# jedison-github/gentun

Measured on AMD Instinct MI355X. Metric: candidates/hour + best val-acc@genN, Genetic-CNN CIFAR-10 1/2/4/8 GPU, higher is better.
Workload: dtype fp32

## Files before the change

### csrc/hip/cnn_args.h

```cpp
#pragma once
#include "common.h"

template <typename F>
static void lds_limit(F* fn, size_t bytes) {
  if (bytes > 65536) (void)hipFuncSetAttribute(reinterpret_cast<const void*>(fn), hipFuncAttributeMaxDynamicSharedMemorySize,
                                         (int)bytes);
}

struct GroupRec {
  int g;
  int in_mask;
  int out_mask;
  int pad;
};

#define GT_MAXSLOT 8

struct ConvArgs {
  const void* in[GT_MAXSLOT];
  const void* mask;
  const int64_t* gather;
  const StepState* st;
  void* out[GT_MAXSLOT];
  const void* out_mask[GT_MAXSLOT];
// ... 17 lines not shown
  int Hr, Wr;
  int wino;
  int wfrag;
  int twopass;
};

__device__ __forceinline__ GroupRec group_rec(const GroupRec* gtab, int y, int n_in, int n_out, int acc,
                                              const void* const* out_mask) {
  if (gtab) return gtab[y];
  GroupRec r;
  r.g = y;
  r.in_mask = (1 << n_in) - 1;
  int rm = 0;
  for (int k = 0; k < n_out; ++k)
    if (out_mask && out_mask[k]) rm |= 1 << k;
  r.out_mask = ((1 << n_out) - 1) | ((acc & 0xff) << 8) | (rm << 16);
  r.pad = 0;
  return r;
}

struct WgradArgs {
  const void* in[GT_MAXSLOT];
  const int64_t* gather;
  const StepState* st;
  const void* dz;
  float* part_w;
  float* part_b;
  const GroupRec* gtab;
  int n_in;
  int G, B, H, W, Cinp, Coutp, KH, KW, S, pps;
  int ngroups;
  int prec;
  int cout_real;
};

__device__ __forceinline__ bool pos_bits(uint32_t h) { return h != 0u && h < 0x8000u; }
```

### csrc/hip/cnn_conv_fast.hip

```cpp
#include "conv_fast_host.h"

FastSwitches g_fast;

static int swap_switch(int& sw, int v) {
  const int old = sw;
  sw = v;
  return old;
}

extern "C" int gt_conv_set_s2in_ct1(int on) { return swap_switch(g_fast.s2in_ct1, on); }

extern "C" int gt_conv_set_regepi(int on) { return swap_switch(g_fast.regepi, on); }

extern "C" int gt_conv_set_smallq(int on) { return swap_switch(g_fast.smallq, on); }

static int smallq_th(const ConvArgs* a, int TH, int THMIN) {
  if (!g_fast.smallq) return TH;
  int th = TH;
  while (th > THMIN && (long)a->ngroups * a->B * (a->H / th) < g_fast.smallq_wg) th >>= 1;
  return th;
}

static bool pk_ok(const ConvArgs* a, int nt) {
  const int last = a->cout_real - 16 * (nt - 1);
// ... 158 lines not shown
      float acc = 0.f;
      for (int sp = 0; sp < a.S; ++sp) acc += pb[(long)sp * a.G * a.Coutp + i];
      pb[i] = acc;
    }
  }
}

extern "C" int gt_wgrad_reduce(const WgradArgs* a, hipStream_t stream) {
  const long n = (long)a->Coutp * a->KH * a->KW * a->Cinp;
  if (n % 4 || a->S < 2) return -1;
  dim3 grid((unsigned)((n / 4 + 255) / 256), a->ngroups);
  hipLaunchKernelGGL(wgrad_reduce_kernel, grid, dim3(256), 0, stream, *a);
  return (int)hipGetLastError();
}

extern "C" int gt_wgrad_set_nb(int nb) { return swap_switch(g_fast.wgrad_nb, nb); }

extern "C" int gt_wgrad_set_nz(int nz) { return swap_switch(g_fast.wgrad_nz, nz); }

static int wgrad_nz(const WgradArgs* a) {
  const int force = g_fast.wgrad_nz;
  if (force == 1 || force == 2 || force == 4 || force == 8) return force;
  const int blocks = a->S * a->ngroups;
  return blocks < 64 ? 4 : blocks < 160 ? 2 : 1;
}

static bool wgrad_pk_ok(const WgradArgs* a, int mt) {
  const int last = a->cout_real - 16 * (mt - 1);
  return a->cout_real > 0 && last >= 1 && last <= 4;
}

static const std::vector<WgradRow>& wgrad_rows() {
  static const std::vector<WgradRow> rows = {
    wgrad_f32<5, 5, 1, 3, 32, 8, 4, 1>(),
    wgrad_f32<3, 3, 3, 3, 32, 4, 4, 1>(),
    wgrad_f32<5, 5, 3, 7, 16, 4, 8, 1>(),
    wgrad_f32<3, 3, 7, 7, 16, 4, 8, 1>(),
    wgrad_f32z<5, 5, 7, 13, 8, 4, 8, 4>(),
    wgrad_f32z<3, 3, 13, 13, 8, 4, 8, 4>(),
    wgrad_f32<5, 5, 1, 8, 32, 4, 4, 1>(),
    wgrad_f32<3, 3, 8, 8, 32, 2, 8, 1>(),
    wgrad_f32z<5, 5, 8, 16, 16, 2, 8, 7>(),
    wgrad_f32z<3, 3, 16, 16, 16, 2, 8, 4>(),
    wgrad_f32z<5, 5, 16, 32, 8, 4, 8, 13>(),
    wgrad_f32z<3, 3, 32, 32, 8, 4, 8, 10>(),
    wgrad_bf16<5, 5, 1, 3, 32, 8, 4, 1>(),
    wgrad_bf16<3, 3, 3, 3, 32, 8, 4, 1>(),
    wgrad_bf16<5, 5, 3, 7, 16, 16, 8, 2>(),
    wgrad_bf16<3, 3, 7, 7, 16, 16, 8, 2>(),
  };
  return rows;
}

static const WgradRow* wgrad_row(int KH, int KW, int Cinp, int Coutp, int H, int W, int prec) {
  for (const std::vector<WgradRow>* rows : {&wgrad_rows(), &wgrad_rows_ext()})
    for (const WgradRow& r : *rows)
      if (KH == r.KH && KW == r.KW && Cinp == r.NCBI * 8 && Coutp == r.NCBO * 8 && W == r.W && prec == r.PREC &&
          H % r.R == 0)
        return &r;
  return nullptr;
}

struct WgradChoice {
  const WgradKernel* k;
  dim3 grid;
  unsigned block;
};

static bool select_wgrad(const WgradArgs* a, WgradChoice* c) {
  const WgradRow* r = wgrad_row(a->KH, a->KW, a->Cinp, a->Coutp, a->H, a->W, a->prec);
  if (!r || a->pps % (r->R * r->W) != 0) return false;
  const int nz = r->NZ ? r->NZ : wgrad_nz(a);
  const int pk = r->PREC == 1 && wgrad_pk_ok(a, (r->NCBO * 8 + 15) / 16) ? 1 : 0;
  int nw = r->NW, nb = 1;
  if (r->NZ == 0 && nz == 2) nb = r->NB;
  else if (r->NZ == 0 && nz == 8) nw = 4;
  else if (nz == 1) nb = (g_fast.wgrad_nb ? g_fast.wgrad_nb : r->NB) == 1 ? 1 : 2;
  for (const WgradKernel& k : r->k)
    if (k.NW == nw && k.NB == nb && k.PK == pk && k.NZ == nz) {
      *c = {&k, dim3(a->S, a->ngroups, nz), (unsigned)nw * 64};
      return true;
    }
  return false;
}

extern "C" int gt_wgrad_fast_band(int KH, int KW, int Cinp, int Coutp, int H, int W, int prec) {
  const WgradRow* r = wgrad_row(KH, KW, Cinp, Coutp, H, W, prec);
  return r ? r->R * r->W : 0;
}

extern "C" int gt_wgrad_fast_splits(int KH, int KW, int Cinp, int Coutp, int H, int W, int prec) {
  (void)KH; (void)KW; (void)Cinp; (void)Coutp; (void)H;
  if (prec == 1) {
    return W >= 32 ? 32 : W <= 8 ? 4 : 8;
  }
  return W >= 32 ? 16 : 3;
}

extern "C" int gt_wgrad_fast(const WgradArgs* a, hipStream_t stream) {
  if (a->prec != 0 && a->prec != 1) return -1;
  WgradChoice c;
  if (!select_wgrad(a, &c)) return -100;
  return launch_fast(c.k->fn, c.grid, c.block, 0, a, stream);
}

struct WgradSel {
  int KH, KW, NCBI, NCBO, W, R, NW, NB, PK, NZ, PREC;
  int gx, gy, gz, block, lds;
};
extern "C" int gt_wgrad_fast_select(const WgradArgs* a, WgradSel* s) {
  WgradChoice c;
  if (!select_wgrad(a, &c)) return 0;
  const WgradKernel& k = *c.k;
  *s = {k.KH, k.KW, k.NCBI, k.NCBO, k.W, k.R, k.NW, k.NB, k.PK, k.NZ, k.PREC,
        (int)c.grid.x, (int)c.grid.y, (int)c.grid.z, (int)c.block, 0};
  return 1;
}
extern "C" size_t gt_sizeof_wgrad_sel() { return sizeof(WgradSel); }

extern "C" int gt_conv_frag_order(int KH, int KW, int NCBI, int W, int prec, int* out, int n) {
  const int NCH = KH * KW * NCBI;
  const bool parts = prec == 1 && NCBI == 7 && W == 16 && KH == 3 && KW == 3;
  for (int e = 0; e < n; ++e) {
    int kk, cb;
    if (e >= NCH) { out[e] = -1; continue; }
    if (parts) {
      const int E0 = KH * KW * 4;
      if (e < E0) { kk = e >> 2; cb = e & 3; }
      else { const int e1 = e - E0; kk = e1 / 3; cb = 4 + e1 - kk * 3; }
    } else {
      kk = e / NCBI; cb = e - kk * NCBI;
    }
    out[e] = kk * NCBI + cb;
  }
  return (NCH + 3) / 4;
}

struct FragSeg {
  const float* w;
  uint16_t* dst;
  const int* order;
  long ps;
  int Q, Cop, Cip, KH, KW;
  int NT, NKS, NCBIc;
  int dgrad;
  int npl;
};

struct FragArgs {
  const FragSeg* segs;
  const int2* blocks;
// ... 51 lines not shown
```

### csrc/hip/conv_fast_host.h

```cpp
#pragma once
#include <initializer_list>
#include <vector>

#include "conv_fast_impl.h"

struct FastSwitches {
  int s2in_ct1 = 1;
  int regepi = 1;
  int smallq = 1;
  long smallq_wg = 300;
  int wgrad_nb = 0;
  int wgrad_nz = 0;
};
extern FastSwitches g_fast;

struct ConvKernel {
  int KH, KW, NCBI, W, TH, NT, NCO, NWV, PREC, PK, RE, CTX, SCH;
  int lds_fwd, lds_bwd;
  int TWO;
  const void* fn;
};

template <int KH, int KW, int NCBI, int W, int TH, int NT, int NCO, int NWV, int PREC, int PK = 0, int RE = 0,
          int CTX = 0, int SCH = 0, int TWO = 0>
// ... 12 lines not shown
  IF_TWO = 16,
};

struct ConvVariant {
  int cond;
  ConvKernel k;
};
typedef std::vector<ConvVariant> ConvVariants;

template <int KH, int KW, int NCBI, int W, int TH, int NT, int NCO, int NWV, int PREC, int PK = 0>
static ConvVariants tile(int cond = 0) {
  ConvVariants v;
  if (PREC == 1 && W % 16 == 0) v.push_back({cond | IF_RE, conv_kernel<KH, KW, NCBI, W, TH, NT, NCO, NWV, PREC, PK, 1>()});
  v.push_back({cond, conv_kernel<KH, KW, NCBI, W, TH, NT, NCO, NWV, PREC, PK, 0>()});
  return v;
}

template <int KH, int KW, int NCBI, int W, int TH, int NT, int NCO, int NWV, int SCH = 1, int TWO = 0>
static ConvVariants ct1(int cond = 0) {
  return {{cond, conv_kernel<KH, KW, NCBI, W, TH, NT, NCO, NWV, 1, 0, 1, 1, SCH, TWO>()}};
}

struct ConvRow {
  int hmod, thmin;
  ConvVariants v;
  ConvRow(int hmod_, int thmin_, std::initializer_list<ConvVariants> parts) : hmod(hmod_), thmin(thmin_) {
    for (const ConvVariants& p : parts) v.insert(v.end(), p.begin(), p.end());
  }
};

struct WgradKernel {
  int KH, KW, NCBI, NCBO, W, R, NW, NB, PK, NZ, PREC;
  const void* fn;
};

template <int KH, int KW, int NCBI, int NCBO, int W, int R, int NW, int NB, int PK = 0, int NZ = 1>
static WgradKernel wgrad_kernel_f32() {
  return {KH, KW, NCBI, NCBO, W, R, NW, NB, PK, NZ, 1,
          reinterpret_cast<const void*>(&wgrad_fast_f32_kernel<KH, KW, NCBI, NCBO, W, R, NW, NB, PK, NZ>)};
}
template <int KH, int KW, int NCBI, int NCBO, int W, int R, int NW, int NB>
static WgradKernel wgrad_kernel_bf16() {
  return {KH, KW, NCBI, NCBO, W, R, NW, NB, 0, 1, 0,
          reinterpret_cast<const void*>(&wgrad_fast_kernel<KH, KW, NCBI, NCBO, W, R, NW, NB>)};
}

struct WgradRow {
  int KH, KW, NCBI, NCBO, W, R, NW, PREC;
  int NB;
  int NZ;
  std::vector<WgradKernel> k;
};

template <int KH, int KW, int NCBI, int NCBO, int W, int R, int NW, int NB>
static WgradRow wgrad_f32() {
  return {KH, KW, NCBI, NCBO, W, R, NW, 1, NB, 0,
          {wgrad_kernel_f32<KH, KW, NCBI, NCBO, W, R, NW, 1, 0>(), wgrad_kernel_f32<KH, KW, NCBI, NCBO, W, R, NW, 1, 1>(),
           wgrad_kernel_f32<KH, KW, NCBI, NCBO, W, R, NW, 2, 0>(), wgrad_kernel_f32<KH, KW, NCBI, NCBO, W, R, NW, 2, 1>(),
           wgrad_kernel_f32<KH, KW, NCBI, NCBO, W, R, NW, NB, 0, 2>(), wgrad_kernel_f32<KH, KW, NCBI, NCBO, W, R, NW, NB, 1, 2>(),
           wgrad_kernel_f32<KH, KW, NCBI, NCBO, W, R, NW, 1, 0, 4>(), wgrad_kernel_f32<KH, KW, NCBI, NCBO, W, R, NW, 1, 1, 4>(),
           wgrad_kernel_f32<KH, KW, NCBI, NCBO, W, R, 4, 1, 0, 8>(), wgrad_kernel_f32<KH, KW, NCBI, NCBO, W, R, 4, 1, 1, 8>()}};
}
template <int KH, int KW, int NCBI, int NCBO, int W, int R, int NW, int NZ>
static WgradRow wgrad_f32z() {
  return {KH, KW, NCBI, NCBO, W, R, NW, 1, 1, NZ,
          {wgrad_kernel_f32<KH, KW, NCBI, NCBO, W, R, NW, 1, 0, NZ>(), wgrad_kernel_f32<KH, KW, NCBI, NCBO, W, R, NW, 1, 1, NZ>()}};
}
template <int KH, int KW, int NCBI, int NCBO, int W, int R, int NW, int NB>
static WgradRow wgrad_bf16() {
  return {KH, KW, NCBI, NCBO, W, R, NW, 0, NB, 1,
          {wgrad_kernel_bf16<KH, KW, NCBI, NCBO, W, R, NW, 1>(), wgrad_kernel_bf16<KH, KW, NCBI, NCBO, W, R, NW, 2>()}};
}

const std::vector<ConvRow>& conv_rows_ext();
const std::vector<WgradRow>& wgrad_rows_ext();
```

### csrc/hip/conv_fast_impl.h

```cpp
#pragma once

#include <algorithm>
#include <cstdio>
#include <cstdlib>
#include <type_traits>

#include "cnn_args.h"


__device__ __forceinline__ int opaque_i(int x) {
  asm volatile("" : "+v"(x));
  return x;
}

template <int KH, int KW, int NCBI, int W, int PREC>
struct S2Parts {
  static constexpr bool on = PREC == 1 && NCBI == 7 && W == 16 && KH == 3 && KW == 3;
  static constexpr int e0 = KH * KW * 4;
};

template <int KH, int KW, int NCBI, int W, int TH, int NT, int NCO, int PREC, int TWO = 0>
struct FastCfg {
  static_assert(!TWO || S2Parts<KH, KW, NCBI, W, PREC>::on, "two-pass staging follows the part-major order");
  static constexpr int NPL = PREC ? GT_NPL_F32 : 1;
// ... 864 lines not shown
        uint4 bfr = tr_pair(x0, x0 + 4 * XROW);
        if (n == NCH / 2 && ones_lane) bfr = make_uint4(0x3f803f80u, 0x3f803f80u, 0x3f803f80u, 0x3f803f80u);
#pragma unroll
        for (int m = 0; m < MT; ++m) acc[m][t] = mfma16(afr[m], bfr, acc[m][t]);
      }
    }
    if (NB == 1 && band + 1 < band1) {
      __syncthreads();
      issue(band + 1, 0);
    }
  }

  const int kq = lane >> 4;
  constexpr int Kdim = NCH * 8;
#pragma unroll
  for (int t = 0; t < TPW; ++t) {
    const int n = wave + NW * t;
    if (n >= NKT) continue;
    const int col = n * 16 + l16;
#pragma unroll
    for (int m = 0; m < MT; ++m)
#pragma unroll
      for (int i = 0; i < 4; ++i) {
        const int co = m * 16 + kq * 4 + i;
        if (co >= a.Coutp) continue;
        if (col < Kdim)
          a.part_w[(((long)s * a.G + g) * a.Coutp + co) * Kdim + col] = acc[m][t][i];
        else if (col == Kdim && a.part_b)
          a.part_b[((long)s * a.G + g) * a.Coutp + co] = acc[m][t][i];
      }
  }
}

template <int KH, int KW, int NCBI, int NCBO, int W, int R, int NW, int NB, int PK = 0, int NZ = 1>
__global__ void __launch_bounds__(NW * 64) wgrad_fast_f32_kernel(WgradArgs a) {
  constexpr int NPL = GT_NPL_F32;
  constexpr int NT_ = NW * 64;
  constexpr int PW = W + KW - 1, PR = R + KH - 1;
  constexpr int NCH = KH * KW * NCBI;
  constexpr int NKT = (NCH + 1 + 1) / 2;
  constexpr int MT = (NCBO * 8 + 15) / 16;
  constexpr int TPW = ((NKT + NZ - 1) / NZ + NW - 1) / NW;
  constexpr int KS = R * W / 32;
  constexpr int XCH = PR * PW * NCBI;
  constexpr int DCH = R * W * NCBO;
  constexpr int XT = (XCH + NT_ - 1) / NT_, DT = (DCH + NT_ - 1) / NT_;
  constexpr int NCBIP0 = NCBI + ((NCBI & 1) ? 0 : 1), NCBOP0 = NCBO + ((NCBO & 1) ? 0 : 1);
  constexpr bool PADOK = (long)NB * NPL * (PR * PW * NCBIP0 + R * W * NCBOP0) * 16 + (long)NB * R * W * 32 <= 160 * 1024;
  constexpr int NCBIP = PADOK ? NCBIP0 : NCBI, NCBOP = PADOK ? NCBOP0 : NCBO;
  constexpr int XCHL = PR * PW * NCBIP, DCHL = R * W * NCBOP;
  constexpr int XROW = NCBIP * 16, DROW = NCBOP * 16;
  auto xslot = [&](int i) {
    if constexpr (NCBIP == NCBI) return i;
    else return (i / NCBI) * NCBIP + i % NCBI;
  };
  auto dslot = [&](int i) {
    if constexpr (NCBOP == NCBO) return i;
    else return (i / NCBO) * NCBOP + i % NCBO;
  };
  constexpr bool MOUT = NZ > 1;
  static_assert(R * W % 32 == 0 && (W == 8 || W == 16 || W == 32), "bands must be whole 32-pixel K-steps");

  __shared__ __attribute__((aligned(16))) uint4 xs[NB][NPL][XCHL];
  __shared__ __attribute__((aligned(16))) uint4 ds[NB][NPL][DCHL];
  constexpr int PKC = 2 * (MT - 1);
  constexpr int PKR = PK ? R * W : 1;
  __shared__ __attribute__((aligned(16))) uint4 dpk[NB][PKR][2];
  static_assert(!PK || PKC < NCBO, "packed tile inside the staged dz chunks");

  const int tid = threadIdx.x, wave = tid >> 6, lane = tid & 63;
  const int s = blockIdx.x;
  const int nz0 = NZ > 1 ? (int)blockIdx.z * NW * TPW : 0;
  const GroupRec gr = group_rec(a.gtab, blockIdx.y, a.n_in, 0, 0, nullptr);
  const int g = gr.g;
  const int nbi = a.H / R;
  const int bps = a.pps / (R * W);
  const int band0 = s * bps;
  const int band1 = min(band0 + bps, a.B * nbi);
  const long img_in = (long)a.H * W * NCBI * 8, img_out = (long)a.H * W * NCBO * 8;
  const long fold_off = (long)g * a.B * img_in;
  const int n_src = a.gather ? 1 : __builtin_popcount(gr.in_mask);
  const float* in0 = static_cast<const float*>(a.in[__builtin_ctz(gr.in_mask | 0x100) & 7]);

  float xr[XT][8], dr[DT][8];
  auto load = [&](int band) {
    const int b = band / nbi, h0 = (band - b * nbi) * R;
    const long boff = fold_off + (long)b * img_in;
    const float* src0 = a.gather ? static_cast<const float*>(a.in[0]) +
                                       a.gather[((long)a.st->cur_step * a.G + g) * a.B + b] * img_in
                                 : in0 + boff;
#pragma unroll
    for (int j = 0; j < XT; ++j) {
      const int i = tid + NT_ * j;
      const int cb = i % NCBI, pix = i / NCBI;
      const int hh = h0 - KH / 2 + pix / PW, ww = pix % PW - KW / 2;
      const bool ok = i < XCH && hh >= 0 && hh < a.H && ww >= 0 && ww < W;
      const long off = ((long)hh * W + ww) * (NCBI * 8) + cb * 8;
      if (n_src == 1) {
#pragma unroll
        for (int e = 0; e < 8; ++e) xr[j][e] = 0.f;
        if (ok) load8f(src0 + off, xr[j]);
      } else {
#pragma unroll
        for (int e = 0; e < 8; ++e) xr[j][e] = 0.f;
        for (int k = 0; k < GT_MAXSLOT; ++k) {
          if (!((gr.in_mask >> k) & 1)) continue;
          float t8[8];
          load8f_or0(static_cast<const float*>(a.in[k]) + boff + off, ok, t8);
#pragma unroll
          for (int e = 0; e < 8; ++e) xr[j][e] += t8[e];
        }
      }
    }
    const float* dsrc = static_cast<const float*>(a.dz) + (long)g * a.B * img_out + (long)b * img_out +
                        (long)h0 * W * NCBO * 8;
#pragma unroll
    for (int j = 0; j < DT; ++j) {
      const int i = tid + NT_ * j;
      if (i < DCH) load8f(dsrc + (long)i * 8, dr[j]);
    }
  };
  auto store = [&](int buf) {
#pragma unroll
    for (int j = 0; j < XT; ++j) {
      const int i = tid + NT_ * j;
      if (i < XCH) split8(xr[j], xs[buf][0][xslot(i)], xs[buf][1][xslot(i)], xs[buf][2][xslot(i)]);
    }
#pragma unroll
    for (int j = 0; j < DT; ++j) {
      const int i = tid + NT_ * j;
      if (i >= DCH) continue;
      uint4 q0, q1, q2;
      split8(dr[j], q0, q1, q2);
      ds[buf][0][dslot(i)] = q0;
      ds[buf][1][dslot(i)] = q1;
      ds[buf][2][dslot(i)] = q2;
      if (PK && i % NCBO == PKC) {
        const int creal = a.cout_real - 16 * (MT - 1);
        uint32_t w[8];
        const uint32_t h0[4] = {q0.x & 0xffffu, q0.x >> 16, q0.y & 0xffffu, q0.y >> 16};
        const uint32_t h1[4] = {q1.x & 0xffffu, q1.x >> 16, q1.y & 0xffffu, q1.y >> 16};
        const uint32_t h2[4] = {q2.x & 0xffffu, q2.x >> 16, q2.y & 0xffffu, q2.y >> 16};
#pragma unroll
        for (int c = 0; c < 4; ++c) {
          w[2 * c] = c < creal ? (h0[c] | (h1[c] << 16)) : 0u;
          w[2 * c + 1] = c < creal ? h2[c] : 0u;
        }
        const int px = i / NCBO;
        dpk[buf][px][0] = make_uint4(w[0], w[1], w[2], w[3]);
        dpk[buf][px][1] = make_uint4(w[4], w[5], w[6], w[7]);
      }
    }
  };

  const int gq = lane >> 4, q = (lane >> 2) & 3, p = lane & 3, l16 = lane & 15;
  const int px0 = 8 * gq + q;
  const int prow = px0 / W, pcol = px0 % W;
  const int xlane = (prow * PW + pcol) * XROW;
  const int dlane = px0 * DROW + p * 8;
  int xoff[TPW];
#pragma unroll
  for (int t = 0; t < TPW; ++t) {
    const int n = nz0 + wave + NW * t;
    int c = 2 * n + (p >> 1);
    if (c >= NCH) c = 0;
    const int kk = c / NCBI, cb = c % NCBI;
    xoff[t] = xlane + ((kk / KW) * PW + (kk % KW)) * XROW + cb * 16 + (p & 1) * 8;
  }
  const bool ones_lane = l16 == (NCH & 1) * 8;

  f32x4_t acc[MT][TPW];
#pragma unroll
  for (int m = 0; m < MT; ++m)
#pragma unroll
    for (int t = 0; t < TPW; ++t) acc[m][t] = (f32x4_t){0.f, 0.f, 0.f, 0.f};

  const bool early = NB == 2 && wave >= NW / 2;
  if (band0 < band1) {
    load(band0);
    store(0);
    if (early && band0 + 1 < band1) load(band0 + 1);
  }
  int cur = 0;
  for (int band = band0; band < band1; ++band, cur ^= (NB - 1)) {
    __syncthreads();
    const bool more = band + 1 < band1;
    if (early) {
      if (more) {
        store(cur ^ 1);
        if (band + 2 < band1) load(band + 2);
      }
    } else if (more) {
      load(band + 1);
    }
#pragma unroll
    for (int ks = 0; ks < KS; ++ks) {
      const int xrow_off = ((ks * 32) / W) * PW * XROW;
      auto load_at = [&](int m, uint4* af) {
        if (PK && m == MT - 1) {
          const char* d0 = reinterpret_cast<const char*>(dpk[cur]) + px0 * 32 + p * 8 + ks * 32 * 32;
          af[0] = tr_pair(d0, d0 + 4 * 32);
          return;
        }
#pragma unroll
        for (int pl = 0; pl < NPL; ++pl) {
          const char* d0 = reinterpret_cast<const char*>(ds[cur][pl]) + dlane + ks * 32 * DROW + m * 32;
          af[pl] = tr_pair(d0, d0 + 4 * DROW);
        }
      };
      auto load_bt = [&](int t, uint4* bfr) {
        const int n = nz0 + wave + NW * t;
#pragma unroll
        for (int pl = 0; pl < NPL; ++pl) {
          const char* x0 = reinterpret_cast<const char*>(xs[cur][pl]) + xrow_off + xoff[t];
          bfr[pl] = tr_pair(x0, x0 + 4 * XROW);
        }
        if (n == NCH / 2 && ones_lane) {
          bfr[0] = make_uint4(0x3f803f80u, 0x3f803f80u, 0x3f803f80u, 0x3f803f80u);
          bfr[1] = bfr[2] = make_uint4(0, 0, 0, 0);
        }
      };
      auto mma = [&](int m, const uint4* af, const uint4* bf, f32x4_t c) {
        if (PK && m == MT - 1) {
          c = mfma16(af[0], bf[2], c);
          c = mfma16(af[0], bf[1], c);
          return mfma16(af[0], bf[0], c);
        }
        return mfma_np<NPL>(af, bf, c);
      };
      if constexpr (MOUT) {
        uint4 bfr[TPW][NPL];
#pragma unroll
        for (int t = 0; t < TPW; ++t) load_bt(t, bfr[t]);
        uint4 af[2][NPL];
        load_at(0, af[0]);
#pragma unroll
        for (int m = 0; m < MT; ++m) {
          if (m + 1 < MT) load_at(m + 1, af[(m + 1) & 1]);
#pragma unroll
          for (int t = 0; t < TPW; ++t)
            if (nz0 + wave + NW * t < NKT) acc[m][t] = mma(m, af[m & 1], bfr[t], acc[m][t]);
        }
      } else {
        uint4 afr[MT][NPL];
#pragma unroll
        for (int m = 0; m < MT; ++m) load_at(m, afr[m]);
        uint4 bfr[2][NPL];
        load_bt(0, bfr[0]);
#pragma unroll
        for (int t = 0; t < TPW; ++t) {
          const int n = wave + NW * t;
          if (t + 1 < TPW) load_bt(t + 1, bfr[(t + 1) & 1]);
          if (n >= NKT) continue;
#pragma unroll
          for (int m = 0; m < MT; ++m) acc[m][t] = mma(m, afr[m], bfr[t & 1], acc[m][t]);
        }
      }
    }
    if (more && !early) {
      if (NB == 1) __syncthreads();
      store(cur ^ (NB - 1));
    }
  }

  const int kq = lane >> 4;
  constexpr int Kdim = NCH * 8;
#pragma unroll
  for (int t = 0; t < TPW; ++t) {
    const int n = nz0 + wave + NW * t;
    if (n >= NKT) continue;
    const int col = n * 16 + l16;
#pragma unroll
    for (int m = 0; m < MT; ++m)
#pragma unroll
      for (int i = 0; i < 4; ++i) {
        const bool pkm = PK && m == MT - 1;
        const int co = pkm ? m * 16 + kq + 4 * i : m * 16 + kq * 4 + i;
        const float v = pkm ? (i == 0 ? acc[m][t][0] + acc[m][t][1] + acc[m][t][2] : 0.f) : acc[m][t][i];
        if (co >= a.Coutp) continue;
        if (col < Kdim)
          a.part_w[(((long)s * a.G + g) * a.Coutp + co) * Kdim + col] = v;
        else if (col == Kdim && a.part_b)
          a.part_b[((long)s * a.G + g) * a.Coutp + co] = v;
      }
  }
}
```

### gentun_amd/models/cnn_hip.py

```python

import math

import numpy as np
import torch

from ..ops import cnn_kernels as K
from ..utils import rng as _rng
from .cnn_engine import FoldJob
from .pop_schedule import PopulationSchedule

WGRAD_STREAMS = 2
POOL_FUSE = True
NATIVE_STEPS = True

WINOGRAD = False

WFRAG = True

TWOPASS = True

EVAL_TWIN_BUDGET = 1 << 30


def pad8(c):
    return (c + 7) // 8 * 8


def round_up(x, m):
    return (x + m - 1) // m * m


def split_planes(w, npl):
    out = torch.empty((npl,) + tuple(w.shape), dtype=torch.bfloat16, device=w.device)
    r = w.float()
    for q in range(npl):
        out[q] = r.to(torch.bfloat16)
        r = r - out[q].float()
    return out


def fast_path_report(plan, dtype="fp32", ngroups=25, B=32, pad_images=True, batch_norm=False):
    prec = K.PREC[dtype]
    h0r, w0r, c0 = plan.input_shape
    kernels, nodes = list(plan.kernels_per_layer), list(plan.nodes)
    ks = [tuple(k) for k in plan.kernel_sizes]
    hw = K.padded_hw(h0r, w0r, len(kernels), batch_norm)
    h0, w0 = hw if pad_images else (h0r, w0r)
    pads = K.stage_channel_pads(c0, kernels, ks, h0, w0, prec, ngroups=ngroups, B=B)
    lib = K.lib()
    layers, generic, fast = [], 0, 0
    cin, cinr = pad8(c0), c0
    for s, (cp, k) in enumerate(zip(pads, ks)):
# ... 521 lines not shown
                if st.pool in self.unpool_fused:
                    continue
                hh, ww, cc = self.shapes[st.inp]
                x1 = self.sched.pool_x1(st)
                self.bwd_ops.append(("pool_bwd", (st.pmask.data_ptr(),
                                                  st.sel.data_ptr(), self.grad[st.pool].data_ptr(),
                                                  self.grad[st.inp].data_ptr(), self.grad[x1].data_ptr(),
                                                  Q * B, B, hh, ww, cc, 1, prec), None))
                continue
            kind, L, rows = rec
            first = L.slots == ["input"]
            if self.bn and L.name not in bn_done:
                bn_done.add(L.name)
                ba = self._bn_args(L, 1)
                ba.y = self.grad[L.name].data_ptr()
                self.bwd_ops.append(("bn_bwd", ba, L))
            if kind == "wgrad":
                wa = K.WgradArgs()
                wslots = L.slots + ([L.xin] if L.xin is not None else [])
                for i, n in enumerate(wslots):
                    wa.inp[i] = self._slot_ptr(n)
                wa.gather = gather_train if first else 0
                if first and self.aug_args is not None:
                    wa.inp[0], wa.gather = self.aug_x.data_ptr(), self.aug_table.data_ptr()
                wa.st = self.state.data_ptr()
                wa.dz = self.grad[L.name].data_ptr()
                wa.part_w, wa.part_b = L.part_w.data_ptr(), L.part_b.data_ptr()
                wa.gtab = self._gtab([(q, im, 0) for q, im in rows]).data_ptr()
                wa.ngroups = len(rows)
                wa.G, wa.B, wa.H, wa.W = Q, B, L.H, L.W
                wa.Cinp, wa.Coutp, wa.KH, wa.KW, wa.S, wa.pps = L.cinp, L.coutp, L.KH, L.KW, L.S, L.pps
                wa.prec = prec
                wa.cout_real = L.cout
                self.bwd_ops.append(("wgrad", wa, L))
            else:
                def dgrad_args(unpool):
                    a = self._conv_args(L, [self.grad[L.name].data_ptr()],
                                        [self._slot_ptr(n, grad=True) for n in L.slots],
                                        [self._slot_ptr(n) for n in L.slots],
                                        L.wUT if L.wino else L.wTF if L.wfragT else L.wT_bf,
                                        None, 0, [(q, 1, of | ((1 << 25) if unpool else 0)) for q, of in rows],
                                        Cinp=L.coutp, Coutp=L.cinp)
                    a.wino = 1 if L.wino else 0
                    a.wfrag = 1 if L.wfragT else 0
                    if unpool:
                        st = pool_stage[L.slots[0]]
                        a.pool_y, a.pool_mask = self.grad[st.inp].data_ptr(), st.pmask.data_ptr()
                        a.unpool_x1 = self.grad[self.sched.pool_x1(st)].data_ptr()
                        a.unpool_sel = st.sel.data_ptr()
                    self._set_twopass(a)
                    return a
                a = None
                if fuse_bwd and len(L.slots) == 1 and L.slots[0] in pool_stage:
                    a = dgrad_args(True)
                    if self.L.gt_conv_fast_probe_any(a):
                        self.unpool_fused.add(L.slots[0])
                    else:
                        a = None
                if a is None:
                    a = dgrad_args(False)
                self.bwd_ops.append(("conv", a, L))
        aa = K.AdamArgs()
        aa.segs, aa.blocks, aa.st = self.adam_segs.data_ptr(), self.adam_blocks.data_ptr(), self.state.data_ptr()
        self.adam_args = aa

    def _build_init_table(self):
# ... 331 lines not shown
```

### gentun_amd/ops/cnn_kernels.py

```python

import ctypes as C
import os

from . import _lib

P = C.c_void_p
I = C.c_int


MAXSLOT = 8

PREC = {"bf16": 0, "fp32": 1}
NPL = {"bf16": 1, "fp32": 3}


class GroupRec(C.Structure):
    _fields_ = [("g", I), ("in_mask", I), ("out_mask", I), ("pad", I)]


class ConvArgs(C.Structure):
    _fields_ = [("inp", P * MAXSLOT), ("mask", P), ("gather", P), ("st", P), ("out", P * MAXSLOT),
                ("out_mask", P * MAXSLOT), ("w", P), ("bias", P), ("gtab", P),
                ("n_in", I), ("n_out", I), ("acc_flags", I), ("relu", I),
                ("G", I), ("B", I), ("H", I), ("W", I), ("Cinp", I), ("Coutp", I), ("KH", I), ("KW", I),
# ... 49 lines not shown
            blocks.extend((len(segs), o) for o in range(0, n, 256))
            segs.append(sg)
        arr = (FragSeg * max(1, len(segs)))(*segs)
        self.segs_t = torch.frombuffer(bytearray(bytes(memoryview(arr).cast("B"))), dtype=torch.uint8).to(device)
        self.blocks_t = torch.tensor(np.asarray(blocks, np.int32).reshape(-1, 2), device=device)
        self.args = FragArgs()
        self.args.segs, self.args.blocks = self.segs_t.data_ptr(), self.blocks_t.data_ptr()
        self.nblocks = len(blocks)

    def run(self, stream):
        if self.nblocks:
            check(lib().gt_conv_wfrag(C.addressof(self.args), self.nblocks, stream), "conv_wfrag")


def frag_planes(master, W, prec=1, dgrad=False):
    import torch
    Q, cop, KH, KW, cip = master.shape
    nt = -(-(cip if dgrad else cop) // 16)
    _, nks = frag_order(KH, KW, (cop if dgrad else cip) // 8, W, prec)
    planes = torch.zeros((3 if prec else 1, Q, nt * nks * 512), dtype=torch.bfloat16, device=master.device)
    tr = FragTransform([(master.contiguous(), planes, W, prec, dgrad)], master.device)
    tr.run(torch.cuda.current_stream(master.device).cuda_stream)
    return planes


def wino_dims(cinp, coutp):
    return -(-coutp // 16) * 16, -(-cinp // 32) * 32


class WgradArgs(C.Structure):
    _fields_ = [("inp", P * MAXSLOT), ("gather", P), ("st", P), ("dz", P), ("part_w", P),
                ("part_b", P), ("gtab", P), ("n_in", I), ("G", I), ("B", I), ("H", I), ("W", I), ("Cinp", I),
                ("Coutp", I), ("KH", I), ("KW", I), ("S", I), ("pps", I), ("ngroups", I), ("prec", I),
                ("cout_real", I)]


class ConvSel(C.Structure):
    _fields_ = [(n, I) for n in ("KH", "KW", "NCBI", "W", "TH", "NT", "NCO", "NWV", "PREC", "PK", "RE", "CTX", "SCH",
                                 "lds_fwd", "lds_bwd", "gx", "gy", "gz", "block", "lds")]


class WgradSel(C.Structure):
    _fields_ = [(n, I) for n in ("KH", "KW", "NCBI", "NCBO", "W", "R", "NW", "NB", "PK", "NZ", "PREC",
                                 "gx", "gy", "gz", "block", "lds")]


class DenseFwdArgs(C.Structure):
    _fields_ = [("x", P), ("wt", P), ("bias", P), ("out", P), ("w2", P), ("plog", P), ("st", P), ("fold_ids", P),
                ("seeds", P), ("G", I), ("B", I), ("Fp", I), ("Up", I), ("drop_p", C.c_float), ("train", I),
                ("seed", C.c_uint), ("C", I), ("prec", I), ("wps", C.c_long), ("row_off", I),
                ("w1", P), ("part", P), ("cnt", P), ("ks", I)]


class HeadArgs(C.Structure):
    _fields_ = [("h", P), ("w2", P), ("b2", P), ("labels", P), ("gather", P), ("st", P), ("dH", P),
                ("gw2", P), ("gb2", P), ("gb1", P), ("eval_out", P), ("dz", P), ("plog", P),
                ("G", I), ("B", I), ("Up", I), ("C", I), ("loss_ce", I), ("drop_scale", C.c_float), ("eval", I),
                ("prec", I), ("valid", P), ("valid_norm", P), ("dHp", P)]


class HeadPredictArgs(C.Structure):
    _fields_ = [("plog", P), ("b2", P), ("logits", P), ("proba", P), ("G", I), ("B", I), ("Up", I), ("C", I)]


class HeadEnsembleArgs(C.Structure):
    _fields_ = [("plog", P), ("b2", P), ("weight", P), ("logits", P), ("proba", P), ("ens", P), ("votes", P),
                ("G", I), ("B", I), ("Up", I), ("C", I)]
# ... 141 lines not shown
        L.gt_step_begin.restype = I
        L.gt_pool_fwd.argtypes = [P, P, P, P, I, I, I, I, I, I, P]
        L.gt_pool_fwd.restype = I
        L.gt_pool_bwd.argtypes = [P, P, P, P, P, P, I, I, I, I, I, I, I, P]
        L.gt_pool_bwd.restype = I
        L.gt_pool_fwd_mask.argtypes = [P, P, P, P, I, I, I, I, I, P, I, P]
        L.gt_pool_fwd_mask.restype = I
        L.gt_pool_bwd_mask.argtypes = [P, P, P, P, P, I, I, I, I, I, I, I, P]
        L.gt_pool_bwd_mask.restype = I
        L.gt_wgrad_set_nb.argtypes = [I]
        L.gt_wgrad_set_nb.restype = I
        L.gt_wgrad_fast_band.argtypes = [I, I, I, I, I, I, I]
        L.gt_wgrad_fast_splits.argtypes = [I, I, I, I, I, I, I]
        L.gt_wgrad_fast_splits.restype = I
        L.gt_wgrad_fast_band.restype = I
        L.gt_conv_fast_probe.argtypes = [C.POINTER(ConvArgs)]
        L.gt_conv_fast_probe.restype = I
        L.gt_conv_fast_probe_any.argtypes = [C.POINTER(ConvArgs)]
        L.gt_conv_fast_probe_any.restype = I
        L.gt_conv_fast_select.argtypes = [C.POINTER(ConvArgs), C.POINTER(ConvSel)]
        L.gt_conv_fast_select.restype = I
        L.gt_conv_fast_twopass.argtypes = [C.POINTER(ConvArgs)]
        L.gt_conv_fast_twopass.restype = I
        L.gt_conv_fast_occupancy.argtypes = [C.POINTER(ConvArgs)]
        L.gt_conv_fast_occupancy.restype = I
        L.gt_wgrad_fast_select.argtypes = [C.POINTER(WgradArgs), C.POINTER(WgradSel)]
        L.gt_wgrad_fast_select.restype = I
        L.gt_sizeof_conv_sel.restype = C.c_size_t
        assert L.gt_sizeof_conv_sel() == C.sizeof(ConvSel), "ConvSel ABI mismatch"
        L.gt_sizeof_wgrad_sel.restype = C.c_size_t
        assert L.gt_sizeof_wgrad_sel() == C.sizeof(WgradSel), "WgradSel ABI mismatch"
        L.gt_wgrad_reduce.argtypes = [C.POINTER(WgradArgs), P]
        L.gt_wgrad_reduce.restype = I
        L.gt_conv_frag_order.argtypes = [I, I, I, I, I, C.POINTER(C.c_int), I]
        L.gt_conv_frag_order.restype = I
        L.gt_conv_wfrag.argtypes = [P, I, P]
        L.gt_conv_wfrag.restype = I
        L.gt_sizeof_frag_seg.restype = C.c_size_t
        assert L.gt_sizeof_frag_seg() == C.sizeof(FragSeg), "FragSeg ABI mismatch"
        L.gt_conv_wino_supported.argtypes = [I, I, I, I]
        L.gt_conv_wino_supported.restype = I
        L.gt_wino_wtrans.argtypes = [P, I, P]
        L.gt_wino_wtrans.restype = I
        L.gt_sizeof_wino_wseg.restype = C.c_size_t
        assert L.gt_sizeof_wino_wseg() == C.sizeof(WinoWSeg), "WinoWSeg ABI mismatch"
        L.gt_conv_set_fast.argtypes = [I]
        L.gt_conv_set_fast.restype = I
        L.gt_dense_fwd_splits.argtypes = [I]
        L.gt_dense_fwd_splits.restype = I
        L.gt_conv_set_smallq.argtypes = [I]
        L.gt_conv_set_smallq.restype = I
        L.gt_conv_set_s2in_ct1.argtypes = [I]
        L.gt_conv_set_s2in_ct1.restype = I
        L.gt_conv_set_imgs.argtypes = [I]
        L.gt_conv_set_imgs.restype = I
        L.gt_glorot_init.argtypes = [C.POINTER(InitArgs), I, P]
        L.gt_glorot_init.restype = I
        L.gt_glorot_ref.argtypes = [C.c_uint64, C.c_uint64, I, C.c_float]
        L.gt_glorot_ref.restype = C.c_float
        L.gt_prog_create.argtypes = [C.POINTER(ProgOp), I, I, I]
        L.gt_prog_create.restype = P
        L.gt_prog_run.argtypes = [P, P, I, C.POINTER(I)]
        L.gt_prog_run.restype = I
        L.gt_prog_destroy.argtypes = [P]
        L.gt_prog_destroy.restype = None
        L.gt_sizeof_prog_op.restype = C.c_size_t
# ... 243 lines not shown
```

Before: 1089.

## Pack four taps per K-tile in first-layer fp32 wgrad kernel

Adds a P4 variant of the fp32 weight-gradient kernel for the first 5x5 conv layer (one input chunk, real channels at most 4). It packs four taps of four channels into each 16-wide K fragment instead of two taps of eight padded channels, which roughly halves the MFMA K-tiles and the input LDS footprint. It also stores the packed last dz tile directly into the main dz buffer. The output column mapping changes and the unused padded weight slots are written as zeros. Selection falls back to the old kernel when no P4 variant matches, and the Python side enables it by default for the first layer.

```diff
diff --git a/csrc/hip/cnn_args.h b/csrc/hip/cnn_args.h
--- a/csrc/hip/cnn_args.h
+++ b/csrc/hip/cnn_args.h
@@ -73,6 +73,7 @@
   int ngroups;
   int prec;
   int cout_real;
+  int pack4;
 };
 
 __device__ __forceinline__ bool pos_bits(uint32_t h) { return h != 0u && h < 0x8000u; }
diff --git a/csrc/hip/cnn_conv_fast.hip b/csrc/hip/cnn_conv_fast.hip
--- a/csrc/hip/cnn_conv_fast.hip
+++ b/csrc/hip/cnn_conv_fast.hip
@@ -214,7 +214,7 @@
 
 static const std::vector<WgradRow>& wgrad_rows() {
   static const std::vector<WgradRow> rows = {
-    wgrad_f32<5, 5, 1, 3, 32, 8, 4, 1>(),
+    wgrad_f32_p4<5, 5, 3, 32, 8, 4, 1>(),
     wgrad_f32<3, 3, 3, 3, 32, 4, 4, 1>(),
     wgrad_f32<5, 5, 3, 7, 16, 4, 8, 1>(),
     wgrad_f32<3, 3, 7, 7, 16, 4, 8, 1>(),
@@ -258,11 +258,12 @@
   if (r->NZ == 0 && nz == 2) nb = r->NB;
   else if (r->NZ == 0 && nz == 8) nw = 4;
   else if (nz == 1) nb = (g_fast.wgrad_nb ? g_fast.wgrad_nb : r->NB) == 1 ? 1 : 2;
-  for (const WgradKernel& k : r->k)
-    if (k.NW == nw && k.NB == nb && k.PK == pk && k.NZ == nz) {
-      *c = {&k, dim3(a->S, a->ngroups, nz), (unsigned)nw * 64};
-      return true;
-    }
+  for (int p4 = a->pack4 ? 1 : 0; p4 >= 0; --p4)
+    for (const WgradKernel& k : r->k)
+      if (k.NW == nw && k.NB == nb && k.PK == pk && k.NZ == nz && k.P4 == p4) {
+        *c = {&k, dim3(a->S, a->ngroups, nz), (unsigned)nw * 64};
+        return true;
+      }
   return false;
 }
 
@@ -299,6 +300,12 @@
   return 1;
 }
 extern "C" size_t gt_sizeof_wgrad_sel() { return sizeof(WgradSel); }
+
+extern "C" int gt_wgrad_fast_pack4(const WgradArgs* a) {
+  WgradChoice c;
+  if ((a->prec != 0 && a->prec != 1) || !select_wgrad(a, &c)) return -1;
+  return c.k->P4;
+}
 
 extern "C" int gt_conv_frag_order(int KH, int KW, int NCBI, int W, int prec, int* out, int n) {
   const int NCH = KH * KW * NCBI;
diff --git a/csrc/hip/conv_fast_host.h b/csrc/hip/conv_fast_host.h
--- a/csrc/hip/conv_fast_host.h
+++ b/csrc/hip/conv_fast_host.h
@@ -68,17 +68,18 @@
 struct WgradKernel {
   int KH, KW, NCBI, NCBO, W, R, NW, NB, PK, NZ, PREC;
   const void* fn;
+  int P4;
 };
 
-template <int KH, int KW, int NCBI, int NCBO, int W, int R, int NW, int NB, int PK = 0, int NZ = 1>
+template <int KH, int KW, int NCBI, int NCBO, int W, int R, int NW, int NB, int PK = 0, int NZ = 1, int P4 = 0>
 static WgradKernel wgrad_kernel_f32() {
   return {KH, KW, NCBI, NCBO, W, R, NW, NB, PK, NZ, 1,
-          reinterpret_cast<const void*>(&wgrad_fast_f32_kernel<KH, KW, NCBI, NCBO, W, R, NW, NB, PK, NZ>)};
+          reinterpret_cast<const void*>(&wgrad_fast_f32_kernel<KH, KW, NCBI, NCBO, W, R, NW, NB, PK, NZ, P4>), P4};
 }
 template <int KH, int KW, int NCBI, int NCBO, int W, int R, int NW, int NB>
 static WgradKernel wgrad_kernel_bf16() {
   return {KH, KW, NCBI, NCBO, W, R, NW, NB, 0, 1, 0,
-          reinterpret_cast<const void*>(&wgrad_fast_kernel<KH, KW, NCBI, NCBO, W, R, NW, NB>)};
+          reinterpret_cast<const void*>(&wgrad_fast_kernel<KH, KW, NCBI, NCBO, W, R, NW, NB>), 0};
 }
 
 struct WgradRow {
@@ -97,6 +98,18 @@
            wgrad_kernel_f32<KH, KW, NCBI, NCBO, W, R, NW, 1, 0, 4>(), wgrad_kernel_f32<KH, KW, NCBI, NCBO, W, R, NW, 1, 1, 4>(),
            wgrad_kernel_f32<KH, KW, NCBI, NCBO, W, R, 4, 1, 0, 8>(), wgrad_kernel_f32<KH, KW, NCBI, NCBO, W, R, 4, 1, 1, 8>()}};
 }
+template <int KH, int KW, int NCBO, int W, int R, int NW, int NB>
+static WgradRow wgrad_f32_p4() {
+  WgradRow r = wgrad_f32<KH, KW, 1, NCBO, W, R, NW, NB>();
+  for (const WgradKernel& k : {
+           wgrad_kernel_f32<KH, KW, 1, NCBO, W, R, NW, 1, 0, 1, 1>(), wgrad_kernel_f32<KH, KW, 1, NCBO, W, R, NW, 1, 1, 1, 1>(),
+           wgrad_kernel_f32<KH, KW, 1, NCBO, W, R, NW, 2, 0, 1, 1>(), wgrad_kernel_f32<KH, KW, 1, NCBO, W, R, NW, 2, 1, 1, 1>(),
+           wgrad_kernel_f32<KH, KW, 1, NCBO, W, R, NW, NB, 0, 2, 1>(), wgrad_kernel_f32<KH, KW, 1, NCBO, W, R, NW, NB, 1, 2, 1>(),
+           wgrad_kernel_f32<KH, KW, 1, NCBO, W, R, NW, 1, 0, 4, 1>(), wgrad_kernel_f32<KH, KW, 1, NCBO, W, R, NW, 1, 1, 4, 1>(),
+           wgrad_kernel_f32<KH, KW, 1, NCBO, W, R, 4, 1, 0, 8, 1>(), wgrad_kernel_f32<KH, KW, 1, NCBO, W, R, 4, 1, 1, 8, 1>()})
+    r.k.push_back(k);
+  return r;
+}
 template <int KH, int KW, int NCBI, int NCBO, int W, int R, int NW, int NZ>
 static WgradRow wgrad_f32z() {
   return {KH, KW, NCBI, NCBO, W, R, NW, 1, 1, NZ,
diff --git a/csrc/hip/conv_fast_impl.h b/csrc/hip/conv_fast_impl.h
--- a/csrc/hip/conv_fast_impl.h
+++ b/csrc/hip/conv_fast_impl.h
@@ -920,13 +920,16 @@
   }
 }
 
-template <int KH, int KW, int NCBI, int NCBO, int W, int R, int NW, int NB, int PK = 0, int NZ = 1>
+template <int KH, int KW, int NCBI, int NCBO, int W, int R, int NW, int NB, int PK = 0, int NZ = 1, int P4 = 0>
 __global__ void __launch_bounds__(NW * 64) wgrad_fast_f32_kernel(WgradArgs a) {
   constexpr int NPL = GT_NPL_F32;
   constexpr int NT_ = NW * 64;
   constexpr int PW = W + KW - 1, PR = R + KH - 1;
   constexpr int NCH = KH * KW * NCBI;
-  constexpr int NKT = (NCH + 1 + 1) / 2;
+  static_assert(!P4 || NCBI == 1, "tap packing: one input chunk");
+  constexpr int NKT = P4 ? (NCH + 1 + 3) / 4 : (NCH + 1 + 1) / 2;
+  constexpr int BIASN = P4 ? NCH / 4 : NCH / 2;
+  constexpr int BIASL = P4 ? (NCH & 3) * 4 : (NCH & 1) * 8;
   constexpr int MT = (NCBO * 8 + 15) / 16;
   constexpr int TPW = ((NKT + NZ - 1) / NZ + NW - 1) / NW;
   constexpr int KS = R * W / 32;
@@ -936,8 +939,8 @@
   constexpr int NCBIP0 = NCBI + ((NCBI & 1) ? 0 : 1), NCBOP0 = NCBO + ((NCBO & 1) ? 0 : 1);
   constexpr bool PADOK = (long)NB * NPL * (PR * PW * NCBIP0 + R * W * NCBOP0) * 16 + (long)NB * R * W * 32 <= 160 * 1024;
   constexpr int NCBIP = PADOK ? NCBIP0 : NCBI, NCBOP = PADOK ? NCBOP0 : NCBO;
-  constexpr int XCHL = PR * PW * NCBIP, DCHL = R * W * NCBOP;
-  constexpr int XROW = NCBIP * 16, DROW = NCBOP * 16;
+  constexpr int XCHL = P4 ? (PR * PW + 1) / 2 : PR * PW * NCBIP, DCHL = R * W * NCBOP;
+  constexpr int XROW = P4 ? 8 : NCBIP * 16, DROW = NCBOP * 16;
   auto xslot = [&](int i) {
     if constexpr (NCBIP == NCBI) return i;
     else return (i / NCBI) * NCBIP + i % NCBI;
@@ -952,7 +955,8 @@
   __shared__ __attribute__((aligned(16))) uint4 xs[NB][NPL][XCHL];
   __shared__ __attribute__((aligned(16))) uint4 ds[NB][NPL][DCHL];
   constexpr int PKC = 2 * (MT - 1);
-  constexpr int PKR = PK ? R * W : 1;
+  constexpr bool PKS = P4 && PK && NCBO == PKC + 1 && NCBOP == NCBO;
+  constexpr int PKR = (PK && !PKS) ? R * W : 1;
   __shared__ __attribute__((aligned(16))) uint4 dpk[NB][PKR][2];
   static_assert(!PK || PKC < NCBO, "packed tile inside the staged dz chunks");
 
@@ -987,7 +991,14 @@
       if (n_src == 1) {
 #pragma unroll
         for (int e = 0; e < 8; ++e) xr[j][e] = 0.f;
-        if (ok) load8f(src0 + off, xr[j]);
+        if constexpr (P4) {
+          if (ok) {
+            const float4 q4 = *reinterpret_cast<const float4*>(src0 + off);
+            xr[j][0] = q4.x; xr[j][1] = q4.y; xr[j][2] = q4.z; xr[j][3] = q4.w;
+          }
+        } else {
+          if (ok) load8f(src0 + off, xr[j]);
+        }
       } else {
 #pragma unroll
         for (int e = 0; e < 8; ++e) xr[j][e] = 0.f;
@@ -1012,7 +1023,16 @@
 #pragma unroll
     for (int j = 0; j < XT; ++j) {
       const int i = tid + NT_ * j;
-      if (i < XCH) split8(xr[j], xs[buf][0][xslot(i)], xs[buf][1][xslot(i)], xs[buf][2][xslot(i)]);
+      if constexpr (P4) {
+        if (i >= XCH) continue;
+        uint4 q0, q1, q2;
+        split8(xr[j], q0, q1, q2);
+        reinterpret_cast<uint2*>(xs[buf][0])[i] = make_uint2(q0.x, q0.y);
+        reinterpret_cast<uint2*>(xs[buf][1])[i] = make_uint2(q1.x, q1.y);
+        reinterpret_cast<uint2*>(xs[buf][2])[i] = make_uint2(q2.x, q2.y);
+      } else {
+        if (i < XCH) split8(xr[j], xs[buf][0][xslot(i)], xs[buf][1][xslot(i)], xs[buf][2][xslot(i)]);
+      }
     }
 #pragma unroll
     for (int j = 0; j < DT; ++j) {
@@ -1020,9 +1040,11 @@
       if (i >= DCH) continue;
       uint4 q0, q1, q2;
       split8(dr[j], q0, q1, q2);
-      ds[buf][0][dslot(i)] = q0;
-      ds[buf][1][dslot(i)] = q1;
-      ds[buf][2][dslot(i)] = q2;
+      if (!PKS || i % NCBO != PKC) {
+        ds[buf][0][dslot(i)] = q0;
+        ds[buf][1][dslot(i)] = q1;
+        ds[buf][2][dslot(i)] = q2;
+      }
       if (PK && i % NCBO == PKC) {
         const int creal = a.cout_real - 16 * (MT - 1);
         uint32_t w[8];
@@ -1035,8 +1057,13 @@
           w[2 * c + 1] = c < creal ? h2[c] : 0u;
         }
         const int px = i / NCBO;
-        dpk[buf][px][0] = make_uint4(w[0], w[1], w[2], w[3]);
-        dpk[buf][px][1] = make_uint4(w[4], w[5], w[6], w[7]);
+        if constexpr (PKS) {
+          ds[buf][0][dslot(i)] = make_uint4(w[0], w[1], w[2], w[3]);
+          ds[buf][1][dslot(i)] = make_uint4(w[4], w[5], w[6], w[7]);
+        } else {
+          dpk[buf][px][0] = make_uint4(w[0], w[1], w[2], w[3]);
+          dpk[buf][px][1] = make_uint4(w[4], w[5], w[6], w[7]);
+        }
       }
     }
   };
@@ -1050,12 +1077,12 @@
 #pragma unroll
   for (int t = 0; t < TPW; ++t) {
     const int n = nz0 + wave + NW * t;
-    int c = 2 * n + (p >> 1);
+    int c = P4 ? 4 * n + p : 2 * n + (p >> 1);
     if (c >= NCH) c = 0;
     const int kk = c / NCBI, cb = c % NCBI;
-    xoff[t] = xlane + ((kk / KW) * PW + (kk % KW)) * XROW + cb * 16 + (p & 1) * 8;
-  }
-  const bool ones_lane = l16 == (NCH & 1) * 8;
+    xoff[t] = xlane + ((kk / KW) * PW + (kk % KW)) * XROW + cb * 16 + (P4 ? 0 : (p & 1) * 8);
+  }
+  const bool ones_lane = l16 == BIASL;
 
   f32x4_t acc[MT][TPW];
 #pragma unroll
@@ -1086,8 +1113,14 @@
       const int xrow_off = ((ks * 32) / W) * PW * XROW;
       auto load_at = [&](int m, uint4* af) {
         if (PK && m == MT - 1) {
-          const char* d0 = reinterpret_cast<const char*>(dpk[cur]) + px0 * 32 + p * 8 + ks * 32 * 32;
-          af[0] = tr_pair(d0, d0 + 4 * 32);
+          if constexpr (PKS) {
+            const char* d0 = reinterpret_cast<const char*>(ds[cur][p >> 1]) + px0 * DROW + PKC * 16 + (p & 1) * 8 +
+                             ks * 32 * DROW;
+            af[0] = tr_pair(d0, d0 + 4 * DROW);
+          } else {
+            const char* d0 = reinterpret_cast<const char*>(dpk[cur]) + px0 * 32 + p * 8 + ks * 32 * 32;
+            af[0] = tr_pair(d0, d0 + 4 * 32);
+          }
           return;
         }
 #pragma unroll
@@ -1103,7 +1136,7 @@
           const char* x0 = reinterpret_cast<const char*>(xs[cur][pl]) + xrow_off + xoff[t];
           bfr[pl] = tr_pair(x0, x0 + 4 * XROW);
         }
-        if (n == NCH / 2 && ones_lane) {
+        if (n == BIASN && ones_lane) {
           bfr[0] = make_uint4(0x3f803f80u, 0x3f803f80u, 0x3f803f80u, 0x3f803f80u);
           bfr[1] = bfr[2] = make_uint4(0, 0, 0, 0);
         }
@@ -1157,7 +1190,7 @@
   for (int t = 0; t < TPW; ++t) {
     const int n = nz0 + wave + NW * t;
     if (n >= NKT) continue;
-    const int col = n * 16 + l16;
+    const int col = P4 ? (4 * n + (l16 >> 2)) * 8 + (l16 & 3) : n * 16 + l16;
 #pragma unroll
     for (int m = 0; m < MT; ++m)
 #pragma unroll
@@ -1166,10 +1199,13 @@
         const int co = pkm ? m * 16 + kq + 4 * i : m * 16 + kq * 4 + i;
         const float v = pkm ? (i == 0 ? acc[m][t][0] + acc[m][t][1] + acc[m][t][2] : 0.f) : acc[m][t][i];
         if (co >= a.Coutp) continue;
-        if (col < Kdim)
-          a.part_w[(((long)s * a.G + g) * a.Coutp + co) * Kdim + col] = v;
-        else if (col == Kdim && a.part_b)
+        if (col < Kdim) {
+          float* pw = a.part_w + (((long)s * a.G + g) * a.Coutp + co) * Kdim + col;
+          *pw = v;
+          if (P4) pw[4] = 0.f;
+        } else if (col == Kdim && a.part_b) {
           a.part_b[((long)s * a.G + g) * a.Coutp + co] = v;
+        }
       }
   }
 }
diff --git a/gentun_amd/models/cnn_hip.py b/gentun_amd/models/cnn_hip.py
--- a/gentun_amd/models/cnn_hip.py
+++ b/gentun_amd/models/cnn_hip.py
@@ -18,6 +18,13 @@
 WFRAG = True
 
 TWOPASS = True
+
+PACK4 = True
+
+
+def pack4_wgrad(first, cin, cinp, prec, fast_on):
+    return 1 if PACK4 and first and cinp == 8 and 1 <= cin <= 4 and prec == 1 and fast_on else 0
+
 
 EVAL_TWIN_BUDGET = 1 << 30
 
@@ -605,6 +612,7 @@
                 wa.Cinp, wa.Coutp, wa.KH, wa.KW, wa.S, wa.pps = L.cinp, L.coutp, L.KH, L.KW, L.S, L.pps
                 wa.prec = prec
                 wa.cout_real = L.cout
+                wa.pack4 = pack4_wgrad(first, L.cin, L.cinp, prec, K.fast_path_on(self.L))
                 self.bwd_ops.append(("wgrad", wa, L))
             else:
                 def dgrad_args(unpool):
diff --git a/gentun_amd/ops/cnn_kernels.py b/gentun_amd/ops/cnn_kernels.py
--- a/gentun_amd/ops/cnn_kernels.py
+++ b/gentun_amd/ops/cnn_kernels.py
@@ -105,7 +105,7 @@
     _fields_ = [("inp", P * MAXSLOT), ("gather", P), ("st", P), ("dz", P), ("part_w", P),
                 ("part_b", P), ("gtab", P), ("n_in", I), ("G", I), ("B", I), ("H", I), ("W", I), ("Cinp", I),
                 ("Coutp", I), ("KH", I), ("KW", I), ("S", I), ("pps", I), ("ngroups", I), ("prec", I),
-                ("cout_real", I)]
+                ("cout_real", I), ("pack4", I)]
 
 
 class ConvSel(C.Structure):
@@ -313,6 +313,12 @@
         assert L.gt_sizeof_wgrad_sel() == C.sizeof(WgradSel), "WgradSel ABI mismatch"
         L.gt_wgrad_reduce.argtypes = [C.POINTER(WgradArgs), P]
         L.gt_wgrad_reduce.restype = I
+        L.gt_wgrad_fast.argtypes = [C.POINTER(WgradArgs), P]
+        L.gt_wgrad_fast.restype = I
+        L.gt_wgrad_fast_pack4.argtypes = [C.POINTER(WgradArgs)]
+        L.gt_wgrad_fast_pack4.restype = I
+        L.gt_wgrad_set_nz.argtypes = [I]
+        L.gt_wgrad_set_nz.restype = I
         L.gt_conv_frag_order.argtypes = [I, I, I, I, I, C.POINTER(C.c_int), I]
         L.gt_conv_frag_order.restype = I
         L.gt_conv_wfrag.argtypes = [P, I, P]
```

Result: faster. 1101, median of 6 (+1.1%).
